# CuzImSlymi/Apertis-LLM

Measured on AMD Instinct MI355X. Metric: train tokens/sec/node (seq=4096), higher is better.
Workload: dtype bf16

## Files before the change

### apertis_llm_amd/csrc/layernorm.hip

```cpp
#include "row_common.h"

namespace {

template <typename TX, typename TO, int IT>
__global__ void __launch_bounds__(256)
gather_ln_fwd_k(const TX *__restrict__ x, const int32_t *__restrict__ row_token,
                const int32_t *__restrict__ offsets, const float *__restrict__ gamma,
                const float *__restrict__ beta, float eps, TO *__restrict__ xg,
                float *__restrict__ mean_o, float *__restrict__ rstd_o, int64_t max_rows, int H, int E) {
  if constexpr (IT <= 4) __builtin_assume(H > 256 * (IT - 1));
  const int lane = threadIdx.x & 63;
  const int64_t r = (int64_t)blockIdx.x * 4 + (threadIdx.x >> 6);
  if (r >= max_rows || (offsets && r >= offsets[E])) return;
  const int e = offsets ? expert_of_row(offsets, E, (int)r) : 0;
  const TX *src = x + (row_token ? (int64_t)row_token[r] : r) * H;
  float4 v[IT];
#pragma unroll
  for (int i = 0; i < IT; ++i) {
    int c = (lane + 64 * i) * 4;
    v[i] = c < H ? load4s<TX>(src + c) : make_float4(0.f, 0.f, 0.f, 0.f);
  }
  float mean, rstd;
  row_stats<IT>(v, lane, H, eps, mean, rstd);
  const float *ga = gamma + (int64_t)e * H, *be = beta + (int64_t)e * H;
// ... 600 lines not shown
    float4 v[IT];
#pragma unroll
    for (int i = 0; i < IT; ++i) {
      const int c = (lane + 64 * i) * 4;
      if (c < H) {
        const float4 a = raw_to_f4(bc[i]), rr = raw_to_f4(rc[i]);
        float e[4] = {a.x, a.y, a.z, a.w};
        if (drop_p > 0.f) {
          bool keep[4];
          drop_keep4(seed, (uint64_t)r * (uint64_t)H + (uint64_t)c, th, keep);
#pragma unroll
          for (int j = 0; j < 4; ++j) e[j] = keep[j] ? e[j] * ks : 0.f;
        }
        v[i] = make_float4(rr.x + e[0], rr.y + e[1], rr.z + e[2], rr.w + e[3]);
        store4<TX>(y + r * H + c, v[i]);
        v[i] = make_float4(to_f32(from_f32<TX>(v[i].x)), to_f32(from_f32<TX>(v[i].y)), to_f32(from_f32<TX>(v[i].z)), to_f32(from_f32<TX>(v[i].w)));
      } else {
        v[i] = make_float4(0.f, 0.f, 0.f, 0.f);
      }
    }
    float mean, rstd;
    row_stats<IT>(v, lane, H, eps, mean, rstd);
#pragma unroll
    for (int i = 0; i < IT; ++i) {
      const int c = (lane + 64 * i) * 4;
      if (c < H) {
        const float4 g4 = sG[lane + 64 * i], b4 = sB[lane + 64 * i];
        const float4 o = make_float4((v[i].x - mean) * rstd * g4.x + b4.x, (v[i].y - mean) * rstd * g4.y + b4.y,
                                     (v[i].z - mean) * rstd * g4.z + b4.z, (v[i].w - mean) * rstd * g4.w + b4.w);
        store4<TO>(xn + r * H + c, o);
        v[i] = make_float4(to_f32(from_f32<TO>(o.x)), to_f32(from_f32<TO>(o.y)), to_f32(from_f32<TO>(o.z)), to_f32(from_f32<TO>(o.w)));
      }
    }
    if (lane == 0) { mean_o[r] = mean; rstd_o[r] = rstd; }
    float rmean, rrstd;
    row_stats<IT>(v, lane, H, reps, rmean, rrstd);
#pragma unroll
    for (int i = 0; i < IT; ++i) {
      const bool in = lane + 64 * i < Q;
      const float4 g4 = in ? sRG[lane + 64 * i] : make_float4(0, 0, 0, 0), b4 = in ? sRB[lane + 64 * i] : make_float4(0, 0, 0, 0);
      v[i] = make_float4((v[i].x - rmean) * rrstd * g4.x + b4.x, (v[i].y - rmean) * rrstd * g4.y + b4.y,
                         (v[i].z - rmean) * rrstd * g4.z + b4.z, (v[i].w - rmean) * rrstd * g4.w + b4.w);
    }
    float acc[NN];
#pragma unroll
    for (int n = 0; n < NN; ++n) {
      float a = 0.f;
#pragma unroll
      for (int i = 0; i < IT; ++i) {
        const float4 wn = lane + 64 * i < Q ? sW[n * Q + lane + 64 * i] : make_float4(0, 0, 0, 0);
        a += (v[i].x * wn.x + v[i].y * wn.y) + (v[i].z * wn.z + v[i].w * wn.w);
      }
      acc[n] = wave_sum(a);
    }
    if (lane < NN) {
      float o = 0.f;
#pragma unroll
      for (int n = 0; n < NN; ++n) if (lane == n) o = acc[n];
      logits[r * NN + lane] = o + (rb ? rb[lane] : 0.f);
    }
    if (lane == 0) { rmean_o[r] = rmean; rrstd_o[r] = rrstd; }
#pragma unroll
    for (int i = 0; i < IT; ++i) { bc[i] = bn[i]; rc[i] = rn[i]; }
  }
}

typedef float v2f __attribute__((ext_vector_type(2)));
__device__ __forceinline__ v2f pk_fma2(v2f a, v2f b, v2f c) { return __builtin_elementwise_fma(a, b, c); }

template <typename TX, int IT, int NN, int MODE>
__global__ void __launch_bounds__(256, MODE == 1 ? 2 : 1)
router_bwd3_k(const TX *__restrict__ x, const float *__restrict__ gamma, const float *__restrict__ beta,
              const float *__restrict__ mean_i, const float *__restrict__ rstd_i, const float *__restrict__ W,
              const float *__restrict__ dlogits, const TX *__restrict__ dres, const TX *__restrict__ grows,
              const int32_t *__restrict__ slot_of, int KS, TX *__restrict__ dx,
              float *__restrict__ part, int64_t T, int H) {
  if constexpr (IT <= 4) __builtin_assume(H > 256 * (IT - 1));
  typedef typename raw4<TX>::type raw_t;
  extern __shared__ __attribute__((aligned(16))) char smem[];
  float4 *sW = reinterpret_cast<float4 *>(smem);
  float4 *red = sW + NN * (H / 4);
  __shared__ float redb[4][SK_MAXN];
  const int lane = threadIdx.x & 63, wv = threadIdx.x >> 6, Q = H / 4;
  for (int i = threadIdx.x; i < NN * Q; i += 256) sW[i] = reinterpret_cast<const float4 *>(W)[i];
  float4 aw[NN][IT], ag[IT], ab[IT], g4[IT], b4[IT];
  float abias = 0.f;
#pragma unroll
  for (int i = 0; i < IT; ++i) {
    const int c = (lane + 64 * i) * 4;
    g4[i] = c < H ? load4<float>(gamma + c) : make_float4(0, 0, 0, 0);
    b4[i] = c < H ? load4<float>(beta + c) : make_float4(0, 0, 0, 0);
    ag[i] = make_float4(0, 0, 0, 0); ab[i] = make_float4(0, 0, 0, 0);
#pragma unroll
    for (int n = 0; n < NN; ++n) aw[n][i] = make_float4(0, 0, 0, 0);
  }
  __syncthreads();
  const int64_t wave = (int64_t)blockIdx.x * 4 + wv, nw = (int64_t)gridDim.x * 4;
  raw_t xc[IT], rc[IT], xn_[IT], rn_[IT];
  raw_t gc[2][IT], gn_[2][IT];
  int sc[2] = {-1, -1}, sn[2] = {-1, -1};
  const bool gath = MODE != 2 && grows != nullptr;
  auto fetch_slots = [&](int64_t r) -> int { return (gath && r < T && lane < KS) ? slot_of[r * KS + lane] : -1; };
  auto slots_of = [&](int v, int (&so)[2]) {
    so[0] = __builtin_amdgcn_readlane(v, 0);
    so[1] = __builtin_amdgcn_readlane(v, 1);
  };
  int slv_n = -1, slv_n2 = -1;
  auto fetch = [&](raw_t (&xo)[IT], raw_t (&ro)[IT], raw_t (&go)[2][IT], const int (&so)[2], int64_t r) {
#pragma unroll
    for (int i = 0; i < IT; ++i) {
      const int c = (lane + 64 * i) * 4;
      const bool ok = c < H && r < T;
      xo[i] = ok ? raw_load(x + r * H + c) : raw_t{};
      ro[i] = (MODE != 2 && ok && dres) ? raw_load(dres + r * H + c) : raw_t{};
#pragma unroll
      for (int k = 0; k < 2; ++k)
        go[k][i] = (gath && ok && so[k] >= 0) ? raw_load(grows + (int64_t)so[k] * H + c) : raw_t{};
    }
  };
  auto fetch_meta = [&](int64_t r) -> float {
    if (r >= T) return 0.f;
    const float *p = lane < NN ? dlogits + r * NN + lane : (lane == NN ? mean_i + r : rstd_i + r);
    return lane < NN + 2 ? *p : 0.f;
  };
  auto lane_val = [](float v, int l) { return __builtin_bit_cast(float, __builtin_amdgcn_readlane(__builtin_bit_cast(int, v), l)); };
  float meta = 0.f, meta_next = 0.f;
  if (wave < T) {
    slots_of(fetch_slots(wave), sc);
    slv_n = fetch_slots(wave + nw);
    fetch(xc, rc, gc, sc, wave);
    meta = fetch_meta(wave);
  }
  for (int64_t r = wave; r < T; r += nw) {
    slv_n2 = fetch_slots(r + 2 * nw);
    slots_of(slv_n, sn);
    fetch(xn_, rn_, gn_, sn, r + nw);
    meta_next = fetch_meta(r + nw);
    float g[NN];
#pragma unroll
    for (int n = 0; n < NN; ++n) g[n] = lane_val(meta, n);
    if (MODE != 1 && lane < NN) abias += meta;
    const float mean = lane_val(meta, NN), rstd = lane_val(meta, NN + 1);
    float4 xh[IT], dn[IT];
    float s1 = 0.f, s2 = 0.f;
#pragma unroll
    for (int i = 0; i < IT; ++i) {
      const bool in = lane + 64 * i < Q;
      const float4 xv = raw_to_f4(xc[i]);
      const v2f mm = {-mean, -mean}, rs = {rstd, rstd};
      v2f xh0 = in ? ((v2f){xv.x, xv.y} + mm) * rs : (v2f){0.f, 0.f}, xh1 = in ? ((v2f){xv.z, xv.w} + mm) * rs : (v2f){0.f, 0.f};
      xh[i] = make_float4(xh0.x, xh0.y, xh1.x, xh1.y);
      const v2f g0 = {g4[i].x, g4[i].y}, g1 = {g4[i].z, g4[i].w};
      const v2f xn0 = pk_fma2(xh0, g0, (v2f){b4[i].x, b4[i].y}), xn1 = pk_fma2(xh1, g1, (v2f){b4[i].z, b4[i].w});
      v2f d0 = {0.f, 0.f}, d1 = {0.f, 0.f};
#pragma unroll
      for (int n = 0; n < NN; ++n) {
        const float4 wn = in ? sW[n * Q + lane + 64 * i] : make_float4(0, 0, 0, 0);
        const v2f gn = {g[n], g[n]};
        if constexpr (MODE != 2) { d0 = pk_fma2(gn, (v2f){wn.x, wn.y}, d0); d1 = pk_fma2(gn, (v2f){wn.z, wn.w}, d1); }
        if constexpr (MODE != 1) {
          v2f a0 = {aw[n][i].x, aw[n][i].y}, a1 = {aw[n][i].z, aw[n][i].w};
          a0 = pk_fma2(gn, xn0, a0); a1 = pk_fma2(gn, xn1, a1);
          aw[n][i] = make_float4(a0.x, a0.y, a1.x, a1.y);
        }
      }
      if constexpr (MODE == 2) continue;
      v2f ag0 = pk_fma2(d0, xh0, (v2f){ag[i].x, ag[i].y}), ag1 = pk_fma2(d1, xh1, (v2f){ag[i].z, ag[i].w});
      ag[i] = make_float4(ag0.x, ag0.y, ag1.x, ag1.y);
      const v2f ab0 = (v2f){ab[i].x, ab[i].y} + d0, ab1 = (v2f){ab[i].z, ab[i].w} + d1;
      ab[i] = make_float4(ab0.x, ab0.y, ab1.x, ab1.y);
      const v2f dn0 = d0 * g0, dn1 = d1 * g1;
      dn[i] = make_float4(dn0.x, dn0.y, dn1.x, dn1.y);
      s1 += (dn[i].x + dn[i].y) + (dn[i].z + dn[i].w);
      s2 += (dn[i].x * xh[i].x + dn[i].y * xh[i].y) + (dn[i].z * xh[i].z + dn[i].w * xh[i].w);
    }
    if constexpr (MODE != 2) {
    const float m1 = wave_sum(s1) * inv_h(H), m2 = wave_sum(s2) * inv_h(H);
#pragma unroll
    for (int i = 0; i < IT; ++i) {
      const int c = (lane + 64 * i) * 4;
      if (c < H) {
        float4 rr = raw_to_f4(rc[i]);
        if (gath) {
          float4 ga = make_float4(0, 0, 0, 0);
#pragma unroll
          for (int k = 0; k < 2; ++k)
            if (sc[k] >= 0) { const float4 gv = raw_to_f4(gc[k][i]); ga.x += gv.x; ga.y += gv.y; ga.z += gv.z; ga.w += gv.w; }
          rr.x += to_f32(from_f32<TX>(ga.x)); rr.y += to_f32(from_f32<TX>(ga.y));
          rr.z += to_f32(from_f32<TX>(ga.z)); rr.w += to_f32(from_f32<TX>(ga.w));
        }
        store4<TX>(dx + r * H + c, make_float4(rstd * (dn[i].x - m1 - xh[i].x * m2) + rr.x, rstd * (dn[i].y - m1 - xh[i].y * m2) + rr.y,
                                                rstd * (dn[i].z - m1 - xh[i].z * m2) + rr.z, rstd * (dn[i].w - m1 - xh[i].w * m2) + rr.w));
      }
    }
    }
#pragma unroll
    for (int i = 0; i < IT; ++i) { xc[i] = xn_[i]; rc[i] = rn_[i]; gc[0][i] = gn_[0][i]; gc[1][i] = gn_[1][i]; }
    sc[0] = sn[0]; sc[1] = sn[1];
    slv_n = slv_n2;
    meta = meta_next;
  }
  if (MODE != 1 && lane < NN) redb[wv][lane] = abias;
  for (int turn = 1; turn < 4; ++turn) {
    __syncthreads();
    if (wv == turn) {
#pragma unroll
      for (int i = 0; i < IT; ++i) {
        const int cq = lane + 64 * i;
        if (cq < Q) {
          if constexpr (MODE != 1) {
#pragma unroll
            for (int n = 0; n < NN; ++n) red[n * Q + cq] = aw[n][i];
          }
          if constexpr (MODE != 2) { red[NN * Q + cq] = ag[i]; red[(NN + 1) * Q + cq] = ab[i]; }
        }
      }
// ... 866 lines not shown
```

### apertis_llm_amd/csrc/ssm_elementwise.hip

```cpp
#include "common.h"

namespace {

template <typename T> __device__ __forceinline__ float4 ld4(const T *p);
template <> __device__ __forceinline__ float4 ld4<float>(const float *p) { return *reinterpret_cast<const float4 *>(p); }
template <> __device__ __forceinline__ float4 ld4<bf16_t>(const bf16_t *p) {
  uint2 u = *reinterpret_cast<const uint2 *>(p);
  return make_float4(__uint_as_float(u.x << 16), __uint_as_float(u.x & 0xffff0000u), __uint_as_float(u.y << 16),
                     __uint_as_float(u.y & 0xffff0000u));
}
template <typename T> __device__ __forceinline__ void st4(T *p, float4 v);
template <> __device__ __forceinline__ void st4<float>(float *p, float4 v) { *reinterpret_cast<float4 *>(p) = v; }
template <> __device__ __forceinline__ void st4<bf16_t>(bf16_t *p, float4 v) {
  typedef __attribute__((ext_vector_type(4))) bf16_t bf4;
  bf4 o = {(bf16_t)v.x, (bf16_t)v.y, (bf16_t)v.z, (bf16_t)v.w};
  *reinterpret_cast<bf4 *>(p) = o;
}

__device__ __forceinline__ float sigmoidf_(float x) { return __builtin_amdgcn_rcpf(1.f + __builtin_amdgcn_exp2f(-x * 1.4426950408889634f)); }
__device__ __forceinline__ float siluf_(float x) { return x * sigmoidf_(x); }
__device__ __forceinline__ float silu_grad(float x) { float s = sigmoidf_(x); return s * (1.f + x * (1.f - s)); }

struct Geo { int CPR, RP; };
__host__ __device__ inline Geo make_geo(int64_t Dn) {
// ... 139 lines not shown
    const uint32_t u[4] = {v.x, v.y, v.z, v.w};
#pragma unroll
    for (int k = 0; k < 4; ++k) { f[2 * k] = __uint_as_float(u[k] << 16); f[2 * k + 1] = __uint_as_float(u[k] & 0xffff0000u); }
  }
  __device__ static __forceinline__ uint4 pack(const float (&f)[8]) {
    bf16_t e[8];
#pragma unroll
    for (int k = 0; k < 8; ++k) e[k] = (bf16_t)f[k];
    uint4 v;
    __builtin_memcpy(&v, e, 16);
    return v;
  }
};

__device__ __forceinline__ void conv_tile_in(char *lds, const char *g, int64_t rs_bytes, int64_t t_first, int64_t L, int nrow,
                                             int PCS, int tid) {
  const int total = nrow * PCS;
  for (int i0 = tid; i0 < total; i0 += 1024) {
    uint4 v[4];
#pragma unroll
    for (int u = 0; u < 4; ++u) {
      const int i = i0 + u * 256;
      const int r = i / PCS, pc = i - r * PCS;
      const int64_t t = t_first + r;
      v[u] = (i < total && t >= 0 && t < L) ? *reinterpret_cast<const uint4 *>(g + t * rs_bytes + pc * 16) : make_uint4(0, 0, 0, 0);
    }
#pragma unroll
    for (int u = 0; u < 4; ++u) {
      const int i = i0 + u * 256;
      if (i < total) *reinterpret_cast<uint4 *>(lds + (size_t)i * 16) = v[u];
    }
  }
}

template <typename T, int KW>
__global__ void __launch_bounds__(256)
dwconv_silu_fwd_tile_k(const T *__restrict__ x, int64_t x_rs, const float *__restrict__ w, const float *__restrict__ bias,
                       T *__restrict__ out, int64_t out_rs, int64_t L, int PCS, int RG, int nchunks) {
  typedef Pc16<T> PC;
  constexpr int EPC = PC::EPC, TT = CONV_TILE_T;
  extern __shared__ __attribute__((aligned(16))) char smem[];
  const int tid = threadIdx.x;
  const int64_t b = blockIdx.x / nchunks;
  const int64_t t0 = (int64_t)(blockIdx.x - b * nchunks) * TT;
  const int rows = (int)min((int64_t)TT, L - t0);
  const int rg = tid / PCS, p = tid - rg * PCS;
  const bool on = rg < RG;
  float wv[EPC][KW], bv[EPC];
  if (on) {
#pragma unroll
    for (int j = 0; j < EPC; ++j) {
      bv[j] = bias[p * EPC + j];
#pragma unroll
      for (int q = 0; q < KW; ++q) wv[j][q] = w[(p * EPC + j) * KW + q];
    }
  }
  conv_tile_in(smem, reinterpret_cast<const char *>(x + b * L * x_rs), x_rs * (int64_t)sizeof(T), t0 - (KW - 1), L, rows + KW - 1,
               PCS, tid);
  __syncthreads();
  if (!on) return;
  const int rowb = PCS * 16;
  char *ob = reinterpret_cast<char *>(out + (b * L + t0) * out_rs) + p * 16;
  for (int r = rg; r < rows; r += RG) {
    float acc[EPC];
#pragma unroll
    for (int j = 0; j < EPC; ++j) acc[j] = bv[j];
#pragma unroll
    for (int q = 0; q < KW; ++q) {
      float f[EPC];
      PC::unpack(*reinterpret_cast<const uint4 *>(smem + (r + q) * rowb + p * 16), f);
#pragma unroll
      for (int j = 0; j < EPC; ++j) acc[j] += wv[j][q] * f[j];
    }
    float o[EPC];
#pragma unroll
    for (int j = 0; j < EPC; ++j) {
      const float s = to_f32(from_f32<T>(acc[j]));
      o[j] = s * sigmoidf_(s);
    }
    *reinterpret_cast<uint4 *>(ob + (int64_t)r * out_rs * (int64_t)sizeof(T)) = PC::pack(o);
  }
}

template <typename T, int KW>
__global__ void __launch_bounds__(256)
dwconv_silu_bwd_k(const T *__restrict__ x, int64_t x_rs, const float *__restrict__ w, const float *__restrict__ bias,
                  const T *__restrict__ dout, int64_t dout_rs, const T *__restrict__ dout2, int64_t dout2_rs,
                  T *__restrict__ dx, int64_t dx_rs,
                  float *__restrict__ dw_part, float *__restrict__ db_part, int64_t B, int64_t L, int Dn) {
  extern __shared__ __attribute__((aligned(16))) char smem[];
  float *red = reinterpret_cast<float *>(smem);
  constexpr int NA = 4 * (KW + 1);
  const Geo g = make_geo(Dn);
  const int rr = threadIdx.x / g.CPR;
  const bool on = rr < g.RP;
  const int64_t runs_per_seq = ceil_div64(L, CONV_TT);
  for (int c0 = 0; c0 < g.CPR; c0 += 256) {
    const int c = c0 + (on ? threadIdx.x - rr * g.CPR : 0);
    float accw[4][KW], accb[4];
#pragma unroll
    for (int j = 0; j < 4; ++j) { accb[j] = 0.f;
#pragma unroll
      for (int q = 0; q < KW; ++q) accw[j][q] = 0.f; }
    if (on && c < g.CPR) {
      float wv[4][KW], bv[4];
#pragma unroll
      for (int j = 0; j < 4; ++j) {
        bv[j] = bias[c * 4 + j];
#pragma unroll
        for (int q = 0; q < KW; ++q) wv[j][q] = w[(c * 4 + j) * KW + q];
      }
      for (int64_t run = (int64_t)blockIdx.x * g.RP + rr; run < B * runs_per_seq; run += (int64_t)gridDim.x * g.RP) {
        const int64_t b = run / runs_per_seq, t0 = (run - b * runs_per_seq) * CONV_TT;
        const T *xb = x + b * L * x_rs + c * 4;
        const T *gb = dout + b * L * dout_rs + c * 4;
        const T *gb2 = dout2 ? dout2 + b * L * dout2_rs + c * 4 : nullptr;
        T *dxb = dx + b * L * dx_rs + c * 4;
        const int64_t t1 = min(t0 + CONV_TT, L);
        float win[KW][4], dp[KW][4];
#pragma unroll
        for (int q = 0; q < KW; ++q)
#pragma unroll
          for (int j = 0; j < 4; ++j) { win[q][j] = 0.f; dp[q][j] = 0.f; }
#pragma unroll
        for (int q = 0; q < KW - 1; ++q) {
          int64_t tt = t0 - (KW - 1) + q;
          if (tt >= 0) { float4 v = ld4<T>(xb + tt * x_rs); win[q + 1][0] = v.x; win[q + 1][1] = v.y; win[q + 1][2] = v.z; win[q + 1][3] = v.w; }
        }
        for (int64_t t = t0; t < t1 + (KW - 1); ++t) {
#pragma unroll
          for (int q = 0; q < KW - 1; ++q)
#pragma unroll
            for (int j = 0; j < 4; ++j) { win[q][j] = win[q + 1][j]; dp[q][j] = dp[q + 1][j]; }
          if (t < L) {
            float4 v = ld4<T>(xb + t * x_rs), gv = ld4<T>(gb + t * dout_rs);
            if (gb2) {
              const float4 g2 = ld4<T>(gb2 + t * dout2_rs);
              gv = make_float4(to_f32(from_f32<T>(gv.x + g2.x)), to_f32(from_f32<T>(gv.y + g2.y)), to_f32(from_f32<T>(gv.z + g2.z)),
                               to_f32(from_f32<T>(gv.w + g2.w)));
            }
            win[KW - 1][0] = v.x; win[KW - 1][1] = v.y; win[KW - 1][2] = v.z; win[KW - 1][3] = v.w;
            const float g_[4] = {gv.x, gv.y, gv.z, gv.w};
#pragma unroll
            for (int j = 0; j < 4; ++j) {
              float s = bv[j];
#pragma unroll
              for (int q = 0; q < KW; ++q) s += wv[j][q] * win[q][j];
              s = to_f32(from_f32<T>(s));
              float d = g_[j] * silu_grad(s);
              dp[KW - 1][j] = d;
              if (t < t1) {
                accb[j] += d;
#pragma unroll
                for (int q = 0; q < KW; ++q) accw[j][q] += d * win[q][j];
              }
            }
          } else {
#pragma unroll
            for (int j = 0; j < 4; ++j) { win[KW - 1][j] = 0.f; dp[KW - 1][j] = 0.f; }
          }
          const int64_t tp = t - (KW - 1);
          if (tp >= t0 && tp < t1) {
            float o[4];
#pragma unroll
            for (int j = 0; j < 4; ++j) {
              float s = 0.f;
#pragma unroll
              for (int q = 0; q < KW; ++q) s += wv[j][q] * dp[KW - 1 - q][j];
              o[j] = s;
            }
            st4<T>(dxb + tp * dx_rs, make_float4(o[0], o[1], o[2], o[3]));
          }
        }
      }
    }
    const int cw = min(g.CPR, 256);
    __syncthreads();
    if (on && c < g.CPR) {
      float *r = red + ((int64_t)rr * cw + (c - c0)) * NA;
#pragma unroll
      for (int j = 0; j < 4; ++j) {
        r[j * (KW + 1) + KW] = accb[j];
#pragma unroll
        for (int q = 0; q < KW; ++q) r[j * (KW + 1) + q] = accw[j][q];
      }
    }
    __syncthreads();
    if (on && rr == 0 && c < g.CPR) {
      for (int j = 0; j < 4; ++j) {
        for (int q = 0; q <= KW; ++q) {
          float s = 0.f;
          for (int r = 0; r < g.RP; ++r) s += red[((int64_t)r * cw + (c - c0)) * NA + j * (KW + 1) + q];
          if (q < KW) dw_part[((int64_t)blockIdx.x * Dn + c * 4 + j) * KW + q] = s;
          else db_part[(int64_t)blockIdx.x * Dn + c * 4 + j] = s;
        }
      }
    }
    __syncthreads();
  }
}

constexpr int CONV_KMAX = 16;

template <typename T>
__global__ void __launch_bounds__(256)
dwconv_silu_fwd_kn(const T *__restrict__ x, int64_t x_rs, const float *__restrict__ w, const float *__restrict__ bias,
                   T *__restrict__ out, int64_t out_rs, int64_t B, int64_t L, int Dn, int k) {
  constexpr int KM = CONV_KMAX;
  const int off = KM - k;
  const Geo g = make_geo(Dn);
  const int rr = threadIdx.x / g.CPR;
  if (rr >= g.RP) return;
  const int64_t runs_per_seq = ceil_div64(L, CONV_TT);
  for (int c = threadIdx.x - rr * g.CPR; c < g.CPR; c += 256) {
    float wv[4][KM], bv[4];
#pragma unroll
    for (int j = 0; j < 4; ++j) {
      bv[j] = bias[c * 4 + j];
#pragma unroll
      for (int m = 0; m < KM; ++m) wv[j][m] = m >= off ? w[(c * 4 + j) * k + (m - off)] : 0.f;
    }
    for (int64_t run = (int64_t)blockIdx.x * g.RP + rr; run < B * runs_per_seq; run += (int64_t)gridDim.x * g.RP) {
      const int64_t b = run / runs_per_seq, t0 = (run - b * runs_per_seq) * CONV_TT;
      const T *xb = x + b * L * x_rs + c * 4;
      T *ob = out + b * L * out_rs + c * 4;
      float win[KM][4];
#pragma unroll
      for (int m = 0; m < KM - 1; ++m) {
        const int64_t tt = t0 - (KM - 1) + m;
        float4 v = (m >= off && tt >= 0) ? ld4<T>(xb + tt * x_rs) : make_float4(0, 0, 0, 0);
        win[m + 1][0] = v.x; win[m + 1][1] = v.y; win[m + 1][2] = v.z; win[m + 1][3] = v.w;
      }
      const int64_t t1 = min(t0 + CONV_TT, L);
      for (int64_t t = t0; t < t1; ++t) {
#pragma unroll
        for (int m = 0; m < KM - 1; ++m)
#pragma unroll
          for (int j = 0; j < 4; ++j) win[m][j] = win[m + 1][j];
        float4 v = ld4<T>(xb + t * x_rs);
        win[KM - 1][0] = v.x; win[KM - 1][1] = v.y; win[KM - 1][2] = v.z; win[KM - 1][3] = v.w;
        float o[4];
#pragma unroll
        for (int j = 0; j < 4; ++j) {
          float s = bv[j];
#pragma unroll
          for (int m = 0; m < KM; ++m)
            if (m >= off) s += wv[j][m] * win[m][j];
          s = to_f32(from_f32<T>(s));
          o[j] = siluf_(s);
        }
        st4<T>(ob + t * out_rs, make_float4(o[0], o[1], o[2], o[3]));
      }
    }
  }
// ... 104 lines not shown
        }
        for (int64_t t = t0; t < t1 + (KM - 1); ++t) {
#pragma unroll
          for (int m = 0; m < KM - 1; ++m)
#pragma unroll
            for (int j = 0; j < 4; ++j) { win[m][j] = win[m + 1][j]; dp[m][j] = dp[m + 1][j]; }
          if (t < te) {
            float4 v = ld4<T>(xb + t * x_rs), gv = ld4<T>(gb + t * dout_rs);
            if (gb2) {
              const float4 g2 = ld4<T>(gb2 + t * dout2_rs);
              gv = make_float4(to_f32(from_f32<T>(gv.x + g2.x)), to_f32(from_f32<T>(gv.y + g2.y)), to_f32(from_f32<T>(gv.z + g2.z)),
                               to_f32(from_f32<T>(gv.w + g2.w)));
            }
            win[KM - 1][0] = v.x; win[KM - 1][1] = v.y; win[KM - 1][2] = v.z; win[KM - 1][3] = v.w;
            const float g_[4] = {gv.x, gv.y, gv.z, gv.w};
#pragma unroll
            for (int j = 0; j < 4; ++j) {
              float s = bv[j];
#pragma unroll
              for (int m = 0; m < KM; ++m)
                if (m >= off) s += wv[j][m] * win[m][j];
              s = to_f32(from_f32<T>(s));
              float d = g_[j] * silu_grad(s);
              dp[KM - 1][j] = d;
              if (t < t1) {
                accb[j] += d;
#pragma unroll
                for (int m = 0; m < KM; ++m)
                  if (m >= off) accw[j][m] += d * win[m][j];
              }
            }
          } else {
#pragma unroll
            for (int j = 0; j < 4; ++j) { win[KM - 1][j] = 0.f; dp[KM - 1][j] = 0.f; }
          }
          const int64_t tp = t - (KM - 1);
          if (tp >= t0) {
            float o[4];
#pragma unroll
            for (int j = 0; j < 4; ++j) {
              float s = 0.f;
#pragma unroll
              for (int m = KM - 1; m >= 0; --m)
                if (m < k) s += wv[j][KM - 1 - m] * dp[m][j];
              o[j] = s;
            }
            st4<T>(dxb + tp * dx_rs, make_float4(o[0], o[1], o[2], o[3]));
          }
        }
      }
    }
    const int cw = min(g.CPR, 256);
    __syncthreads();
    if (on && c < g.CPR) {
      float *r = red + ((int64_t)rr * cw + (c - c0)) * NA;
#pragma unroll
      for (int j = 0; j < 4; ++j) {
        r[j * (k + 1) + k] = accb[j];
#pragma unroll
        for (int m = 0; m < KM; ++m)
          if (m >= off) r[j * (k + 1) + (m - off)] = accw[j][m];
      }
    }
    __syncthreads();
    if (on && rr == 0 && c < g.CPR) {
      for (int j = 0; j < 4; ++j) {
        for (int q = 0; q <= k; ++q) {
          float s = 0.f;
          for (int r = 0; r < g.RP; ++r) s += red[((int64_t)r * cw + (c - c0)) * NA + j * (k + 1) + q];
          if (q < k) dw_part[((int64_t)blockIdx.x * Dn + c * 4 + j) * k + q] = s;
          else db_part[(int64_t)blockIdx.x * Dn + c * 4 + j] = s;
        }
      }
    }
    __syncthreads();
  }
}

__global__ void __launch_bounds__(1024)
colsum_rows_k(const float *__restrict__ in, float *__restrict__ out, int64_t rows, int64_t cols) {
  colsum_block(in, 0, rows, cols, [&](int64_t c, float t) { out[c] = t; });
}

template <typename TX, typename TR>
__global__ void __launch_bounds__(256)
dropout_add_fwd_k(const TX *__restrict__ x, const TR *__restrict__ res, TR *__restrict__ y, int64_t n4, float drop_p,
                  uint64_t seed) {
  const float ks = drop_p > 0.f ? 1.f / (1.f - drop_p) : 1.f;
  const uint32_t th = (uint32_t)(drop_p * 65536.f);
  for (int64_t v = (int64_t)blockIdx.x * blockDim.x + threadIdx.x; v < n4; v += (int64_t)gridDim.x * blockDim.x) {
    float4 a = ld4<TX>(x + v * 4), r = ld4<TR>(res + v * 4);
    float e[4] = {a.x, a.y, a.z, a.w};
    if (drop_p > 0.f) {
#pragma unroll
      for (int j = 0; j < 4; ++j) e[j] = drop_keep(seed, 0, v * 4 + j, 0, th) ? e[j] * ks : 0.f;
    }
    st4<TR>(y + v * 4, make_float4(r.x + e[0], r.y + e[1], r.z + e[2], r.w + e[3]));
  }
}

template <typename TG, typename TX>
__global__ void __launch_bounds__(256)
dropout_bwd_k(const TG *__restrict__ g, TX *__restrict__ dx, int64_t n4, float drop_p, uint64_t seed) {
  const float ks = drop_p > 0.f ? 1.f / (1.f - drop_p) : 1.f;
  const uint32_t th = (uint32_t)(drop_p * 65536.f);
  for (int64_t v = (int64_t)blockIdx.x * blockDim.x + threadIdx.x; v < n4; v += (int64_t)gridDim.x * blockDim.x) {
    float4 a = ld4<TG>(g + v * 4);
    float e[4] = {a.x, a.y, a.z, a.w};
    if (drop_p > 0.f) {
#pragma unroll
      for (int j = 0; j < 4; ++j) e[j] = drop_keep(seed, 0, v * 4 + j, 0, th) ? e[j] * ks : 0.f;
    }
    st4<TX>(dx + v * 4, make_float4(e[0], e[1], e[2], e[3]));
  }
}

template <typename TO>
__global__ void __launch_bounds__(256)
cast_transpose_k(const float *__restrict__ src, TO *__restrict__ dst, TO *__restrict__ dstT, int R, int C, int ld_dst,
                 int ld_dstT) {
  __shared__ float tile[64][65];
  const int64_t e = blockIdx.z;
  const int r0 = blockIdx.y * 64, c0 = blockIdx.x * 64;
  const float *s = src + e * (int64_t)R * C;
  const int tx = threadIdx.x & 63, ty = threadIdx.x >> 6;
  for (int i = ty; i < 64; i += 4) {
    int r = r0 + i, c = c0 + tx;
    float v = (r < R && c < C) ? s[(int64_t)r * C + c] : 0.f;
    tile[i][tx] = v;
    if (dst && r < R && c < ld_dst) dst[e * (int64_t)R * ld_dst + (int64_t)r * ld_dst + c] = from_f32<TO>(v);
  }
  __syncthreads();
  if (dstT)
    for (int i = ty; i < 64; i += 4) {
      int c = c0 + i, r = r0 + tx;
      if (r < ld_dstT && c < C) dstT[e * (int64_t)C * ld_dstT + (int64_t)c * ld_dstT + r] = from_f32<TO>(tile[tx][i]);
    }
}

template <typename TO> struct out4;
template <> struct out4<bf16_t> {
  __device__ static __forceinline__ void store(bf16_t *p, float a, float b, float c, float d) {
    typedef __attribute__((ext_vector_type(4))) bf16_t bf4;
    const bf4 v = {(bf16_t)a, (bf16_t)b, (bf16_t)c, (bf16_t)d};
    *reinterpret_cast<bf4 *>(p) = v;
  }
};
template <> struct out4<float> {
  __device__ static __forceinline__ void store(float *p, float a, float b, float c, float d) {
    *reinterpret_cast<float4 *>(p) = make_float4(a, b, c, d);
  }
};
template <typename TO>
__global__ void __launch_bounds__(256)
cast_transpose4_k(const float *__restrict__ src, TO *__restrict__ dst, TO *__restrict__ dstT, int R, int C, int ld_dst,
                  int ld_dstT) {
  __shared__ float tile[64][65];
  const int64_t e = blockIdx.z;
  const int r0 = blockIdx.y * 64, c0 = blockIdx.x * 64;
  const float *s = src + e * (int64_t)R * C;
  const int q = threadIdx.x & 15, g = threadIdx.x >> 4;
#pragma unroll
  for (int i = 0; i < 4; ++i) {
    const int rl = g + 16 * i, r = r0 + rl, c = c0 + q * 4;
    float4 v = make_float4(0.f, 0.f, 0.f, 0.f);
    if (r < R && c < C) v = *reinterpret_cast<const float4 *>(s + (int64_t)r * C + c);
// ... 126 lines not shown
  hipLaunchKernelGGL(colsum_rows_k, dim3((unsigned)ceil_div64(Dn, 64)), dim3(1024), 0, st, dD_part, dD, (int64_t)nblk, Dn);
  return apertis_check_launch();
}

#define CONV_DISPATCH(k_, dt_, ...)                                                             \
  do {                                                                                          \
    if ((dt_) == APERTIS_F32) { typedef float T;                                                \
      if ((k_) == 2) { constexpr int KW = 2; __VA_ARGS__; } else if ((k_) == 3) { constexpr int KW = 3; __VA_ARGS__; } \
      else if ((k_) == 4) { constexpr int KW = 4; __VA_ARGS__; } else return APERTIS_ERR_UNSUPPORTED; }  \
    else if ((dt_) == APERTIS_BF16) { typedef bf16_t T;                                         \
      if ((k_) == 2) { constexpr int KW = 2; __VA_ARGS__; } else if ((k_) == 3) { constexpr int KW = 3; __VA_ARGS__; } \
      else if ((k_) == 4) { constexpr int KW = 4; __VA_ARGS__; } else return APERTIS_ERR_UNSUPPORTED; }  \
    else return APERTIS_ERR_ARG;                                                                \
  } while (0)

#define CONV_TYPES(dt_, ...)                                                                    \
  do {                                                                                          \
    if ((dt_) == APERTIS_F32) { typedef float T; __VA_ARGS__; }                                 \
    else if ((dt_) == APERTIS_BF16) { typedef bf16_t T; __VA_ARGS__; }                          \
    else return APERTIS_ERR_ARG;                                                                \
  } while (0)

extern "C" int apertis_dwconv_silu_fwd(const void *x, int64_t x_rs, const float *w, const float *bias, void *out,
                                       int64_t out_rs, int64_t B, int64_t L, int64_t Dn, int64_t k, int dtype_io,
                                       void *stream) {
  if (!x || !w || !bias || !out || B < 0 || L < 0) return APERTIS_ERR_ARG;
  if (!rows_ok(Dn) || (x_rs | out_rs) % 4) return APERTIS_ERR_UNSUPPORTED;
  if (B == 0 || L == 0) return APERTIS_OK;
  hipStream_t st = (hipStream_t)stream;
  if (conv_tile_ok(B, L, Dn, k, dtype_io, {x, out}, {x_rs, out_rs})) {
    const int64_t epc = dtype_io == APERTIS_BF16 ? 8 : 4;
    const int PCS = (int)(Dn / epc), RG = 256 / PCS, nchunks = (int)ceil_div64(L, CONV_TILE_T);
    const size_t lds = (size_t)conv_tile_lds(Dn, k, dtype_io);
    CONV_DISPATCH(k, dtype_io, launch_lds(dwconv_silu_fwd_tile_k<T, KW>, dim3((unsigned)(B * nchunks)), dim3(256), lds, st,
                                          (const T *)x, x_rs, w, bias, (T *)out, out_rs, L, PCS, RG, nchunks));
    return apertis_check_launch();
  }
  dim3 grid(conv_blocks(B, L, Dn)), block(256);
  if (k > 4 && k <= CONV_KMAX) {
    CONV_TYPES(dtype_io, hipLaunchKernelGGL(dwconv_silu_fwd_kn<T>, grid, block, 0, st, (const T *)x, x_rs, w, bias, (T *)out,
                                            out_rs, B, L, (int)Dn, (int)k));
    return apertis_check_launch();
  }
  CONV_DISPATCH(k, dtype_io, hipLaunchKernelGGL((dwconv_silu_fwd_k<T, KW>), grid, block, 0, st, (const T *)x, x_rs, w, bias,
                                                (T *)out, out_rs, B, L, (int)Dn));
  return apertis_check_launch();
}

extern "C" int apertis_dwconv_silu_start_fwd(const void *x, int64_t x_rs, const float *w, const float *bias, const int32_t *start,
                                             void *out, int64_t out_rs, int64_t B, int64_t L, int64_t Dn, int64_t k, int dtype_io,
                                             void *stream) {
  if (!x || !w || !bias || !start || !out || B < 0 || L < 0) return APERTIS_ERR_ARG;
  if (dtype_io != APERTIS_F32 && dtype_io != APERTIS_BF16) return APERTIS_ERR_ARG;
  if (!rows_ok(Dn) || (x_rs | out_rs) % 4 || x_rs < Dn || out_rs < Dn || k < 2 || k > CONV_KMAX) return APERTIS_ERR_UNSUPPORTED;
  const uintptr_t piece = dtype_io == APERTIS_BF16 ? 8 : 16;
  if ((uintptr_t)x % piece || (uintptr_t)out % piece) return APERTIS_ERR_UNSUPPORTED;
  if (B == 0 || L == 0) return APERTIS_OK;
  const int CPR = (int)(Dn / 4), CB = std::min(CPR, 64);
  const int64_t nchunks = ceil_div64(L, CONV_TILE_T), ncb = ceil_div64(CPR, CB);
  if (nchunks >= 0x7fffffffLL || B * nchunks * ncb >= 0x7fffffffLL) return APERTIS_ERR_UNSUPPORTED;
  const size_t lds = (size_t)(CONV_TILE_T + 2 * k - 1) * CB * sizeof(float4);
  CONV_TYPES(dtype_io, launch_lds(dwconv_silu_start_k<T>, dim3((unsigned)(B * nchunks * ncb)), dim3(256), lds, (hipStream_t)stream,
                                  (const T *)x, x_rs, w, bias, start, (T *)out, out_rs, L, CPR, (int)k, CB, (int)nchunks, (int)ncb));
  return apertis_check_launch();
}

extern "C" int apertis_dwconv_silu_bwd2(const void *x, int64_t x_rs, const float *w, const float *bias, const void *dout,
                                        int64_t dout_rs, const void *dout2, int64_t dout2_rs, void *dx, int64_t dx_rs,
                                        float *dw_part, float *db_part, float *dw, float *db, int64_t B, int64_t L, int64_t Dn,
                                        int64_t k, int dtype_io, void *stream) {
  if (!x || !w || !bias || !dout || !dx || !dw_part || !db_part || !dw || !db || B < 0 || L < 0) return APERTIS_ERR_ARG;
  if (!dout2) dout2_rs = 0;
  if (!rows_ok(Dn) || (x_rs | dout_rs | dout2_rs | dx_rs) % 4 || k < 2 || k > CONV_KMAX) return APERTIS_ERR_UNSUPPORTED;
  hipStream_t st = (hipStream_t)stream;
  const int nblk = conv_blocks(B, L, Dn);
  {
    Geo g = make_geo(Dn);
    size_t lds = (size_t)g.RP * std::min(g.CPR, 256) * 4 * (k + 1) * sizeof(float);
    dim3 grid(nblk), block(256);
    if (k > 4) {
      CONV_TYPES(dtype_io, launch_lds(dwconv_silu_bwd_kn<T>, grid, block, lds, st, (const T *)x, x_rs, w, bias, (const T *)dout,
                                      dout_rs, (const T *)dout2, dout2_rs, (T *)dx, dx_rs, dw_part, db_part, B, L, (int)Dn, (int)k));
    } else {
      CONV_DISPATCH(k, dtype_io, launch_lds(dwconv_silu_bwd_k<T, KW>, grid, block, lds, st, (const T *)x, x_rs, w,
                                                    bias, (const T *)dout, dout_rs, (const T *)dout2, dout2_rs, (T *)dx, dx_rs,
                                                    dw_part, db_part, B, L, (int)Dn));
    }
  }
  hipLaunchKernelGGL(colsum_rows_k, dim3((unsigned)ceil_div64(Dn * k, 64)), dim3(1024), 0, st, dw_part, dw, (int64_t)nblk,
                     Dn * k);
  hipLaunchKernelGGL(colsum_rows_k, dim3((unsigned)ceil_div64(Dn, 64)), dim3(1024), 0, st, db_part, db, (int64_t)nblk, Dn);
  return apertis_check_launch();
}

extern "C" int apertis_dwconv_silu_bwd(const void *x, int64_t x_rs, const float *w, const float *bias, const void *dout,
                                       int64_t dout_rs, void *dx, int64_t dx_rs, float *dw_part, float *db_part,
                                       float *dw, float *db, int64_t B, int64_t L, int64_t Dn, int64_t k, int dtype_io,
                                       void *stream) {
  return apertis_dwconv_silu_bwd2(x, x_rs, w, bias, dout, dout_rs, nullptr, 0, dx, dx_rs, dw_part, db_part, dw, db, B, L, Dn, k,
                                  dtype_io, stream);
}

extern "C" int apertis_cast_transpose(const float *src, void *dst, void *dstT, int64_t E, int64_t R, int64_t C,
                                      int64_t ld_dst, int64_t ld_dstT, int dtype_out, void *stream) {
  if (!src || (!dst && !dstT) || E <= 0 || R <= 0 || C <= 0) return APERTIS_ERR_ARG;
  if (ld_dst == 0) ld_dst = C;
  if (ld_dstT == 0) ld_dstT = R;
  if (ld_dst < C || ld_dst > ceil_div64(C, 64) * 64 || ld_dstT < R || ld_dstT > ceil_div64(R, 64) * 64) return APERTIS_ERR_ARG;
  if (R > 0x3fffffff || C > 0x3fffffff || E > 65535 || ceil_div64(R, 64) > 65535) return APERTIS_ERR_UNSUPPORTED;
  hipStream_t st = (hipStream_t)stream;
  dim3 grid((unsigned)ceil_div64(C, 64), (unsigned)ceil_div64(R, 64), (unsigned)E), block(256);
  const bool vec4 = C % 4 == 0 && ld_dst % 4 == 0 && ld_dstT % 4 == 0 && (R * C) % 4 == 0 && ((uintptr_t)src) % 16 == 0 &&
                    ((uintptr_t)dst) % 16 == 0 && ((uintptr_t)dstT) % 16 == 0;
#define CT_GO(KERN, TO) hipLaunchKernelGGL(KERN<TO>, grid, block, 0, st, src, (TO *)dst, (TO *)dstT, (int)R, (int)C, (int)ld_dst, (int)ld_dstT)
  if (dtype_out == APERTIS_BF16) {
    if (vec4) CT_GO(cast_transpose4_k, bf16_t); else CT_GO(cast_transpose_k, bf16_t);
  } else if (dtype_out == APERTIS_F32) {
    if (vec4) CT_GO(cast_transpose4_k, float); else CT_GO(cast_transpose_k, float);
  } else {
    return APERTIS_ERR_ARG;
  }
#undef CT_GO
  return apertis_check_launch();
}

extern "C" int64_t apertis_weight_prep_entry_bytes(void) { return (int64_t)sizeof(WPEntry); }
extern "C" int apertis_weight_prep(const void *table, int64_t n_entries, int64_t total_tiles, void *stream) {
  if (!table || n_entries <= 0 || total_tiles <= 0 || n_entries > 0x7fffffff || total_tiles > 0x7fffffff) return APERTIS_ERR_ARG;
  hipLaunchKernelGGL(weight_prep_k, dim3((unsigned)total_tiles), dim3(256), 0, (hipStream_t)stream, (const WPEntry *)table,
                     (int)n_entries);
  return apertis_check_launch();
}

extern "C" int apertis_colsum_f32(const float *in, float *out, int64_t rows, int64_t cols, void *stream) {
  if (!in || !out || rows < 0 || cols <= 0) return APERTIS_ERR_ARG;
  hipLaunchKernelGGL(colsum_rows_k, dim3((unsigned)ceil_div64(cols, 64)), dim3(1024), 0, (hipStream_t)stream, in, out, rows,
                     cols);
  return apertis_check_launch();
}

extern "C" int apertis_dropout_add_fwd(const void *x, const void *res, void *y, int64_t n, float drop_p, uint64_t seed,
                                       int dtype_x, int dtype_res, void *stream) {
  if (!x || !res || !y || n < 0 || drop_p < 0.f || drop_p >= 1.f) return APERTIS_ERR_ARG;
  if (n % 4) return APERTIS_ERR_UNSUPPORTED;
  if (n == 0) return APERTIS_OK;
  hipStream_t st = (hipStream_t)stream;
  const int64_t nb = std::min<int64_t>(ceil_div64(n / 4, 256), 8192);
  dim3 grid((unsigned)nb), block(256);
  if (dtype_x == APERTIS_BF16 && dtype_res == APERTIS_F32)
    hipLaunchKernelGGL((dropout_add_fwd_k<bf16_t, float>), grid, block, 0, st, (const bf16_t *)x, (const float *)res, (float *)y, n / 4, drop_p, seed);
  else if (dtype_x == APERTIS_F32 && dtype_res == APERTIS_F32)
    hipLaunchKernelGGL((dropout_add_fwd_k<float, float>), grid, block, 0, st, (const float *)x, (const float *)res, (float *)y, n / 4, drop_p, seed);
  else if (dtype_x == APERTIS_BF16 && dtype_res == APERTIS_BF16)
    hipLaunchKernelGGL((dropout_add_fwd_k<bf16_t, bf16_t>), grid, block, 0, st, (const bf16_t *)x, (const bf16_t *)res, (bf16_t *)y, n / 4, drop_p, seed);
  else
    return APERTIS_ERR_UNSUPPORTED;
  return apertis_check_launch();
}

extern "C" int apertis_dropout_bwd(const void *g, void *dx, int64_t n, float drop_p, uint64_t seed, int dtype_g,
                                   int dtype_x, void *stream) {
  if (!g || !dx || n < 0 || drop_p < 0.f || drop_p >= 1.f) return APERTIS_ERR_ARG;
  if (n % 4) return APERTIS_ERR_UNSUPPORTED;
  if (n == 0) return APERTIS_OK;
  hipStream_t st = (hipStream_t)stream;
  const int64_t nb = std::min<int64_t>(ceil_div64(n / 4, 256), 8192);
  dim3 grid((unsigned)nb), block(256);
  if (dtype_g == APERTIS_F32 && dtype_x == APERTIS_BF16)
    hipLaunchKernelGGL((dropout_bwd_k<float, bf16_t>), grid, block, 0, st, (const float *)g, (bf16_t *)dx, n / 4, drop_p, seed);
  else if (dtype_g == APERTIS_F32 && dtype_x == APERTIS_F32)
    hipLaunchKernelGGL((dropout_bwd_k<float, float>), grid, block, 0, st, (const float *)g, (float *)dx, n / 4, drop_p, seed);
  else if (dtype_g == APERTIS_BF16 && dtype_x == APERTIS_BF16)
    hipLaunchKernelGGL((dropout_bwd_k<bf16_t, bf16_t>), grid, block, 0, st, (const bf16_t *)g, (bf16_t *)dx, n / 4, drop_p, seed);
  else
// ... 4 lines not shown
```

Measured before the change: 398,300.

## Add prefetched MODE-2 router backward loop and software-pipelined dwconv backward

In the router backward kernel, MODE 2 gets its own loop that skips loading W into shared memory and keeps several rows of x and metadata in flight through a register ring, using sched barriers so the next loads overlap the current row's accumulation. The dwconv-SiLU backward kernel is split on a PAIR template flag and now prefetches a group of input and gradient rows ahead in registers, with launch-bounds occupancy hints added. The two column-sum launches for dw and db are merged into one kernel. These target memory latency and launch overhead, at the cost of more registers and some redundant clamped loads at row ends.

```diff
diff --git a/apertis_llm_amd/csrc/layernorm.hip b/apertis_llm_amd/csrc/layernorm.hip
--- a/apertis_llm_amd/csrc/layernorm.hip
+++ b/apertis_llm_amd/csrc/layernorm.hip
@@ -706,7 +706,8 @@
   float4 *red = sW + NN * (H / 4);
   __shared__ float redb[4][SK_MAXN];
   const int lane = threadIdx.x & 63, wv = threadIdx.x >> 6, Q = H / 4;
-  for (int i = threadIdx.x; i < NN * Q; i += 256) sW[i] = reinterpret_cast<const float4 *>(W)[i];
+  if constexpr (MODE != 2)
+    for (int i = threadIdx.x; i < NN * Q; i += 256) sW[i] = reinterpret_cast<const float4 *>(W)[i];
   float4 aw[NN][IT], ag[IT], ab[IT], g4[IT], b4[IT];
   float abias = 0.f;
 #pragma unroll
@@ -749,13 +750,69 @@
   };
   auto lane_val = [](float v, int l) { return __builtin_bit_cast(float, __builtin_amdgcn_readlane(__builtin_bit_cast(int, v), l)); };
   float meta = 0.f, meta_next = 0.f;
-  if (wave < T) {
+  if constexpr (MODE == 2) {
+    constexpr int RA = sizeof(TX) == 4 && IT == 4 ? 2 : 4;
+    raw_t xq[RA][IT];
+    float mq[RA];
+    const float *mbase = lane < NN ? dlogits + lane : (lane == NN ? mean_i : rstd_i);
+    const int64_t mstride = lane < NN ? NN : 1;
+    auto fetch_row = [&](raw_t (&xo)[IT], float &mo, int64_t r) {
+      const int64_t rl = r < T ? r : T - 1;
+#pragma unroll
+      for (int i = 0; i < IT; ++i) {
+        const int c = (lane + 64 * i) * 4;
+        xo[i] = raw_load(x + rl * H + (c < H ? c : 0));
+      }
+      mo = mbase[rl * mstride];
+    };
+    const int64_t wave_u = (int64_t)blockIdx.x * 4 + __builtin_amdgcn_readfirstlane(wv);
+    if (wave_u < T) {
+#pragma unroll
+      for (int d = 0; d < RA; ++d) fetch_row(xq[d], mq[d], wave_u + d * nw);
+    }
+    for (int64_t r0 = wave_u; r0 < T; r0 += RA * nw) {
+#pragma unroll
+      for (int d = 0; d < RA; ++d) {
+        const int64_t r = r0 + d * nw;
+        float4 xv[IT];
+#pragma unroll
+        for (int i = 0; i < IT; ++i) xv[i] = raw_to_f4(xq[d][i]);
+        const float mr = mq[d];
+        float g[NN];
+#pragma unroll
+        for (int n = 0; n < NN; ++n) g[n] = lane_val(mr, n);
+        const float mean = lane_val(mr, NN), rstd = lane_val(mr, NN + 1);
+        if (r < T && lane < NN) abias += mr;
+        __builtin_amdgcn_sched_barrier(0);
+        fetch_row(xq[d], mq[d], r + RA * nw);
+        __builtin_amdgcn_sched_barrier(0);
+        if (r >= T) continue;
+#pragma unroll
+        for (int i = 0; i < IT; ++i) {
+          const bool in = lane + 64 * i < Q;
+          const v2f mm = {-mean, -mean}, rs = {rstd, rstd};
+          const v2f xh0 = in ? ((v2f){xv[i].x, xv[i].y} + mm) * rs : (v2f){0.f, 0.f};
+          const v2f xh1 = in ? ((v2f){xv[i].z, xv[i].w} + mm) * rs : (v2f){0.f, 0.f};
+          const v2f g0 = {g4[i].x, g4[i].y}, g1 = {g4[i].z, g4[i].w};
+          const v2f xn0 = pk_fma2(xh0, g0, (v2f){b4[i].x, b4[i].y}), xn1 = pk_fma2(xh1, g1, (v2f){b4[i].z, b4[i].w});
+#pragma unroll
+          for (int n = 0; n < NN; ++n) {
+            const v2f gn = {g[n], g[n]};
+            v2f a0 = {aw[n][i].x, aw[n][i].y}, a1 = {aw[n][i].z, aw[n][i].w};
+            a0 = pk_fma2(gn, xn0, a0); a1 = pk_fma2(gn, xn1, a1);
+            aw[n][i] = make_float4(a0.x, a0.y, a1.x, a1.y);
+          }
+        }
+      }
+    }
+  }
+  if (MODE != 2 && wave < T) {
     slots_of(fetch_slots(wave), sc);
     slv_n = fetch_slots(wave + nw);
     fetch(xc, rc, gc, sc, wave);
     meta = fetch_meta(wave);
   }
-  for (int64_t r = wave; r < T; r += nw) {
+  for (int64_t r = wave; MODE != 2 && r < T; r += nw) {
     slv_n2 = fetch_slots(r + 2 * nw);
     slots_of(slv_n, sn);
     fetch(xn_, rn_, gn_, sn, r + nw);
diff --git a/apertis_llm_amd/csrc/ssm_elementwise.hip b/apertis_llm_amd/csrc/ssm_elementwise.hip
--- a/apertis_llm_amd/csrc/ssm_elementwise.hip
+++ b/apertis_llm_amd/csrc/ssm_elementwise.hip
@@ -245,15 +245,28 @@
   }
 }
 
-template <typename T, int KW>
-__global__ void __launch_bounds__(256)
+template <typename T> struct raw4c { typedef float4 type; };
+template <> struct raw4c<bf16_t> { typedef uint2 type; };
+template <typename T> __device__ __forceinline__ typename raw4c<T>::type ld_raw(const T *p) {
+  return *reinterpret_cast<const typename raw4c<T>::type *>(p);
+}
+__device__ __forceinline__ float4 raw_f4(const float4 &v) { return v; }
+__device__ __forceinline__ float4 raw_f4(const uint2 &u) {
+  return make_float4(__uint_as_float(u.x << 16), __uint_as_float(u.x & 0xffff0000u), __uint_as_float(u.y << 16),
+                     __uint_as_float(u.y & 0xffff0000u));
+}
+
+template <typename T, int KW, bool PAIR>
+__global__ void __launch_bounds__(256, KW == 2 ? 4 : 3)
 dwconv_silu_bwd_k(const T *__restrict__ x, int64_t x_rs, const float *__restrict__ w, const float *__restrict__ bias,
                   const T *__restrict__ dout, int64_t dout_rs, const T *__restrict__ dout2, int64_t dout2_rs,
                   T *__restrict__ dx, int64_t dx_rs,
                   float *__restrict__ dw_part, float *__restrict__ db_part, int64_t B, int64_t L, int Dn) {
   extern __shared__ __attribute__((aligned(16))) char smem[];
   float *red = reinterpret_cast<float *>(smem);
-  constexpr int NA = 4 * (KW + 1);
+  constexpr int NA = 4 * (KW + 1), NW = CONV_TT + KW - 1;
+  constexpr int PG = sizeof(T) == 2 ? (KW == 4 ? 3 : 4) : (KW == 3 ? 2 : 1);
+  typedef typename raw4c<T>::type raw_t;
   const Geo g = make_geo(Dn);
   const int rr = threadIdx.x / g.CPR;
   const bool on = rr < g.RP;
@@ -277,62 +290,86 @@
         const int64_t b = run / runs_per_seq, t0 = (run - b * runs_per_seq) * CONV_TT;
         const T *xb = x + b * L * x_rs + c * 4;
         const T *gb = dout + b * L * dout_rs + c * 4;
-        const T *gb2 = dout2 ? dout2 + b * L * dout2_rs + c * 4 : nullptr;
+        const T *gb2 = PAIR ? dout2 + b * L * dout2_rs + c * 4 : nullptr;
         T *dxb = dx + b * L * dx_rs + c * 4;
         const int64_t t1 = min(t0 + CONV_TT, L);
+        const int n1 = (int)(t1 - t0), nw = n1 + (KW - 1), nl = (int)(min(t1 + (KW - 1), L) - t0);
         float win[KW][4], dp[KW][4];
 #pragma unroll
         for (int q = 0; q < KW; ++q)
 #pragma unroll
           for (int j = 0; j < 4; ++j) { win[q][j] = 0.f; dp[q][j] = 0.f; }
+        raw_t fx[PG], fg[PG], fh[PG];
+        const T *lx = xb + t0 * x_rs, *lg = gb + t0 * dout_rs, *lh = PAIR ? gb2 + t0 * dout2_rs : nullptr;
+        T *sx = dxb + t0 * dx_rs;
+        int il = 0;
+        auto load = [&](raw_t &xr, raw_t &gr, raw_t &hr) {
+          xr = ld_raw<T>(lx);
+          gr = ld_raw<T>(lg);
+          if constexpr (PAIR) hr = ld_raw<T>(lh); else hr = raw_t{};
+          const bool more = ++il < nl;
+          lx += more ? x_rs : 0;
+          lg += more ? dout_rs : 0;
+          if constexpr (PAIR) lh += more ? dout2_rs : 0;
+        };
+#pragma unroll
+        for (int i = 0; i < PG; ++i) load(fx[i], fg[i], fh[i]);
 #pragma unroll
         for (int q = 0; q < KW - 1; ++q) {
           int64_t tt = t0 - (KW - 1) + q;
           if (tt >= 0) { float4 v = ld4<T>(xb + tt * x_rs); win[q + 1][0] = v.x; win[q + 1][1] = v.y; win[q + 1][2] = v.z; win[q + 1][3] = v.w; }
         }
-        for (int64_t t = t0; t < t1 + (KW - 1); ++t) {
-#pragma unroll
-          for (int q = 0; q < KW - 1; ++q)
-#pragma unroll
-            for (int j = 0; j < 4; ++j) { win[q][j] = win[q + 1][j]; dp[q][j] = dp[q + 1][j]; }
-          if (t < L) {
-            float4 v = ld4<T>(xb + t * x_rs), gv = ld4<T>(gb + t * dout_rs);
-            if (gb2) {
-              const float4 g2 = ld4<T>(gb2 + t * dout2_rs);
-              gv = make_float4(to_f32(from_f32<T>(gv.x + g2.x)), to_f32(from_f32<T>(gv.y + g2.y)), to_f32(from_f32<T>(gv.z + g2.z)),
-                               to_f32(from_f32<T>(gv.w + g2.w)));
+        for (int ig = 0; ig < NW; ig += PG) {
+#pragma unroll
+          for (int s = 0; s < PG; ++s) {
+            const int i = ig + s;
+            if (i >= NW) break;
+            const raw_t xr = fx[s], gr = fg[s], hr = fh[s];
+            load(fx[s], fg[s], fh[s]);
+            if (i >= nw) continue;
+#pragma unroll
+            for (int q = 0; q < KW - 1; ++q)
+#pragma unroll
+              for (int j = 0; j < 4; ++j) { win[q][j] = win[q + 1][j]; dp[q][j] = dp[q + 1][j]; }
+            if (i < nl) {
+              float4 v = raw_f4(xr), gv = raw_f4(gr);
+              if constexpr (PAIR) {
+                const float4 g2 = raw_f4(hr);
+                gv = make_float4(to_f32(from_f32<T>(gv.x + g2.x)), to_f32(from_f32<T>(gv.y + g2.y)), to_f32(from_f32<T>(gv.z + g2.z)),
+                                 to_f32(from_f32<T>(gv.w + g2.w)));
+              }
+              win[KW - 1][0] = v.x; win[KW - 1][1] = v.y; win[KW - 1][2] = v.z; win[KW - 1][3] = v.w;
+              const float g_[4] = {gv.x, gv.y, gv.z, gv.w};
+#pragma unroll
+              for (int j = 0; j < 4; ++j) {
+                float s = bv[j];
+#pragma unroll
+                for (int q = 0; q < KW; ++q) s += wv[j][q] * win[q][j];
+                s = to_f32(from_f32<T>(s));
+                float d = g_[j] * silu_grad(s);
+                dp[KW - 1][j] = d;
+                if (i < n1) {
+                  accb[j] += d;
+#pragma unroll
+                  for (int q = 0; q < KW; ++q) accw[j][q] += d * win[q][j];
+                }
+              }
+            } else {
+#pragma unroll
+              for (int j = 0; j < 4; ++j) { win[KW - 1][j] = 0.f; dp[KW - 1][j] = 0.f; }
             }
-            win[KW - 1][0] = v.x; win[KW - 1][1] = v.y; win[KW - 1][2] = v.z; win[KW - 1][3] = v.w;
-            const float g_[4] = {gv.x, gv.y, gv.z, gv.w};
-#pragma unroll
-            for (int j = 0; j < 4; ++j) {
-              float s = bv[j];
-#pragma unroll
-              for (int q = 0; q < KW; ++q) s += wv[j][q] * win[q][j];
-              s = to_f32(from_f32<T>(s));
-              float d = g_[j] * silu_grad(s);
-              dp[KW - 1][j] = d;
-              if (t < t1) {
-                accb[j] += d;
-#pragma unroll
-                for (int q = 0; q < KW; ++q) accw[j][q] += d * win[q][j];
+            if (i >= KW - 1) {
+              float o[4];
+#pragma unroll
+              for (int j = 0; j < 4; ++j) {
+                float s = 0.f;
+#pragma unroll
+                for (int q = 0; q < KW; ++q) s += wv[j][q] * dp[KW - 1 - q][j];
+                o[j] = s;
               }
+              st4<T>(sx, make_float4(o[0], o[1], o[2], o[3]));
+              sx += dx_rs;
             }
-          } else {
-#pragma unroll
-            for (int j = 0; j < 4; ++j) { win[KW - 1][j] = 0.f; dp[KW - 1][j] = 0.f; }
-          }
-          const int64_t tp = t - (KW - 1);
-          if (tp >= t0 && tp < t1) {
-            float o[4];
-#pragma unroll
-            for (int j = 0; j < 4; ++j) {
-              float s = 0.f;
-#pragma unroll
-              for (int q = 0; q < KW; ++q) s += wv[j][q] * dp[KW - 1 - q][j];
-              o[j] = s;
-            }
-            st4<T>(dxb + tp * dx_rs, make_float4(o[0], o[1], o[2], o[3]));
           }
         }
       }
@@ -603,6 +640,34 @@
   colsum_block(in, 0, rows, cols, [&](int64_t c, float t) { out[c] = t; });
 }
 
+__global__ void __launch_bounds__(1024)
+colsum_rows_pair_k(const float *__restrict__ a, float *__restrict__ out_a, int64_t cols_a, int nb_a, const float *__restrict__ b,
+                   float *__restrict__ out_b, int64_t cols_b, int64_t rows) {
+  __shared__ float part[16][64];
+  const bool first = (int)blockIdx.x < nb_a;
+  const float *__restrict__ in = first ? a : b;
+  const int64_t cols = first ? cols_a : cols_b;
+  const int lane = threadIdx.x & 63, seg = threadIdx.x >> 6;
+  const int64_t c = (int64_t)(first ? blockIdx.x : blockIdx.x - nb_a) * 64 + lane;
+  float s = 0.f;
+  if (c < cols) {
+    int64_t r = seg;
+    for (; r + 48 < rows; r += 64) {
+      float a0 = in[r * cols + c], a1 = in[(r + 16) * cols + c], a2 = in[(r + 32) * cols + c], a3 = in[(r + 48) * cols + c];
+      s += (a0 + a1) + (a2 + a3);
+    }
+    for (; r < rows; r += 16) s += in[r * cols + c];
+  }
+  part[seg][lane] = s;
+  __syncthreads();
+  if (seg == 0 && c < cols) {
+    float t = 0.f;
+#pragma unroll
+    for (int i = 0; i < 16; ++i) t += part[i][lane];
+    (first ? out_a : out_b)[c] = t;
+  }
+}
+
 template <typename TX, typename TR>
 __global__ void __launch_bounds__(256)
 dropout_add_fwd_k(const TX *__restrict__ x, const TR *__restrict__ res, TR *__restrict__ y, int64_t n4, float drop_p,
@@ -895,14 +960,16 @@
       CONV_TYPES(dtype_io, launch_lds(dwconv_silu_bwd_kn<T>, grid, block, lds, st, (const T *)x, x_rs, w, bias, (const T *)dout,
                                       dout_rs, (const T *)dout2, dout2_rs, (T *)dx, dx_rs, dw_part, db_part, B, L, (int)Dn, (int)k));
     } else {
-      CONV_DISPATCH(k, dtype_io, launch_lds(dwconv_silu_bwd_k<T, KW>, grid, block, lds, st, (const T *)x, x_rs, w,
-                                                    bias, (const T *)dout, dout_rs, (const T *)dout2, dout2_rs, (T *)dx, dx_rs,
-                                                    dw_part, db_part, B, L, (int)Dn));
-    }
-  }
-  hipLaunchKernelGGL(colsum_rows_k, dim3((unsigned)ceil_div64(Dn * k, 64)), dim3(1024), 0, st, dw_part, dw, (int64_t)nblk,
-                     Dn * k);
-  hipLaunchKernelGGL(colsum_rows_k, dim3((unsigned)ceil_div64(Dn, 64)), dim3(1024), 0, st, db_part, db, (int64_t)nblk, Dn);
+#define CONV_BWD(PAIR_) CONV_DISPATCH(k, dtype_io, launch_lds(dwconv_silu_bwd_k<T, KW, PAIR_>, grid, block, lds, st, (const T *)x, \
+                                                              x_rs, w, bias, (const T *)dout, dout_rs, (const T *)dout2, dout2_rs, \
+                                                              (T *)dx, dx_rs, dw_part, db_part, B, L, (int)Dn))
+      if (dout2) CONV_BWD(true); else CONV_BWD(false);
+#undef CONV_BWD
+    }
+  }
+  const int nb_w = (int)ceil_div64(Dn * k, 64), nb_b = (int)ceil_div64(Dn, 64);
+  hipLaunchKernelGGL(colsum_rows_pair_k, dim3((unsigned)(nb_w + nb_b)), dim3(1024), 0, st, dw_part, dw, Dn * k, nb_w, db_part, db,
+                     Dn, (int64_t)nblk);
   return apertis_check_launch();
 }
 
```

Result: no change. 401,300 (median of 6 runs) (+0.7%).
